# quinnchr-personal/Continuum-Mechanics-MFEM

Measured on AMD Instinct MI355X. Metric: DoF-iter/s (CG, 3D p=2 hex convection-diffusion) + achieved HBM GB/s, higher is better.
Workload: dtype f64; 1 GPU; 64x64x64 hex, H1 p=2, PA D+C+M (kinds=7), Jacobi-CG 100 it/step; dofs=2146689, elements=262144, parallelism=single, series=weak: an n^3 slab per rank

## Files before the change

continuum-mechanics-mfem_amd/csrc/brick_core.hpp:

```cpp
#pragma once
#include <hip/hip_runtime.h>

#include <cstdint>

#include "pa_core.hpp"

#ifndef CDFEM_PS8_SKIP
#define CDFEM_PS8_SKIP 1
#endif

namespace cdfem {

struct BrickGeom {
    int nbx, nby, nbz;
    int Lx, Ly, Lz;
    int xcd;
    int bz0, bzs;
    const uint8_t *bess;
    int stag = 0, stag_round = 0;
};

__device__ __forceinline__ void brick_stagger(const BrickGeom &g)
{
    if (g.stag == 0 || gridDim.x < 2u * (unsigned)g.stag_round) return;
    const unsigned wb = blockIdx.x;
    if (wb < (unsigned)g.stag_round && ((wb >> (g.stag & 15)) & 1u))
// ... 12 lines not shown
}
__device__ __forceinline__ void bstore(__amdgpu_buffer_rsrc_t r, uint32_t off, double v)
{
    __builtin_amdgcn_raw_buffer_store_b64(__builtin_bit_cast(u32x2_t, v), r, off, 0, 0);
}

template <int S, int STEP = 64>
struct PatchWalk {
    int x, y, z;
    __device__ __forceinline__ explicit PatchWalk(unsigned t) : x((int)(t % S)), y((int)((t / S) % S)), z((int)(t / (S * S))) {}
    __device__ __forceinline__ void next()
    {
        constexpr int dx = STEP % S, dy = (STEP / S) % S, dz = STEP / (S * S);
        x += dx;
        const int cx = x >= S ? 1 : 0;
        x -= S & -cx;
        y += dy + cx;
        const int cy = y >= S ? 1 : 0;
        y -= S & -cy;
        z += dz + cy;
    }
};

__device__ __forceinline__ int opaque(int v)
{
    asm volatile("" : "+v"(v));
    return v;
}

template <int S, int SZ = S>
__device__ __forceinline__ double patch_sum8(__amdgpu_buffer_rsrc_t bp, const BrickGeom &g, int gx, int gy, int gz)
{
    constexpr int s1 = S - 1, sz1 = SZ - 1;
    const int qx = min(gx / s1, g.nbx - 1), qy = min(gy / s1, g.nby - 1), qz = min(gz / sz1, g.nbz - 1);
    const int px = gx - qx * s1, py = gy - qy * s1, pz = gz - qz * sz1;
    const bool fx = px == 0 && qx > 0, fy = py == 0 && qy > 0, fz = pz == 0 && qz > 0;
    const uint32_t R = (uint32_t)g.nbx * S, A = (uint32_t)g.nby * S * R;
    const uint32_t P = (((uint32_t)qz * SZ + pz) * g.nby + qy) * S * R + (uint32_t)py * R + (uint32_t)qx * S + px;
    bool ax = true, ay = true, az = true;
    if constexpr (CDFEM_PS8_SKIP) {
        ax = __builtin_amdgcn_ballot_w64(fx) != 0;
        ay = __builtin_amdgcn_ballot_w64(fy) != 0;
        az = __builtin_amdgcn_ballot_w64(fz) != 0;
    }
    double t[8];
#pragma unroll
    for (int k = 0; k < 8; ++k) {
        const int sz = (k >> 2) & 1 ? 0 : 1, sy = (k >> 1) & 1 ? 0 : 1, sx = k & 1 ? 0 : 1;
        const bool ok = (!sx || fx) && (!sy || fy) && (!sz || fz);
        const uint32_t o = P - (uint32_t)sx - (uint32_t)sy * R - (uint32_t)sz * A;
        t[k] = 0.0;
        if ((!sx || ax) && (!sy || ay) && (!sz || az)) t[k] = bload(bp, ok ? 8u * o : kOOB);
    }
    double q = 0.0;
#pragma unroll
    for (int k = 0; k < 8; ++k) q += t[k];
    return q;
}

hipError_t launch_hobrick_um(cdfem_ctx *c, const BrickGeom &g, const double *r, const double *dinv, const double *d_old,
                             double *d_new, double *x);

struct GmPatchSrc {
    const double *pb;
    const uint8_t *ess;
    const double *x;
    BrickGeom g;
    FastDiv fdx, fdxy;
    int S;
};
bool brick_mult_pb_on(const cdfem_ctx *c);
GmPatchSrc gm_patch_src(const cdfem_ctx *c, const double *x);

}
```

continuum-mechanics-mfem_amd/csrc/brick_kernels.hip:

```cpp
#include <hip/hip_runtime.h>

#include <type_traits>
#include <vector>
#include <algorithm>
#include <cmath>

#include "cdfem_internal.hpp"
#include "brick_core.hpp"
#include "pa_core.hpp"
#include "reduce.hpp"

#ifndef CDFEM_BRICK_LDS
#define CDFEM_BRICK_LDS 1
#endif

namespace cdfem {

__device__ __forceinline__ int brick_id(const BrickGeom &g)
{
    if (!g.xcd) return blockIdx.x;
    const unsigned G = gridDim.x, b = blockIdx.x, x = b % 8, k = b / 8, q = G / 8, r = G % 8;
    return (int)(x * q + (x < r ? x : r) + k);
}

template <int S, int STEP = 64>
struct LatWalk {
    int x, y, z;
    uint32_t gid;
    __device__ __forceinline__ LatWalk(unsigned t, uint32_t g0, uint32_t Lx, uint32_t Lxy)
        : x((int)(t % S)), y((int)((t / S) % S)), z((int)(t / (S * S)))
    {
        gid = g0 + (uint32_t)x + Lx * (uint32_t)y + Lxy * (uint32_t)z;
    }
    __device__ __forceinline__ void next(uint32_t dgid, uint32_t cxd, uint32_t cyd)
    {
        constexpr int dx = STEP % S, dy = (STEP / S) % S, dz = STEP / (S * S);
        x += dx;
        const int cx = x >= S ? 1 : 0;
        x -= S & -cx;
        y += dy + cx;
        const int cy = y >= S ? 1 : 0;
        y -= S & -cy;
        z += dz + cy;
        gid += dgid + (cxd & (uint32_t)-cx) + (cyd & (uint32_t)-cy);
    }
};

__device__ __forceinline__ int bsel(bool c, int a, int b)
{
    const int m = -(int)c;
    return (a & m) | (b & ~m);
}
template <int S>
__device__ __forceinline__ int face_index(int a, int b, int c)
{
    constexpr int ring = 4 * S - 4;
    const int cap = a + S * b;
    const int mid = bsel(b == 0, a, bsel(b == S - 1, S + 2 * (S - 2) + a, S + 2 * (b - 1) + (int)(a == S - 1)));
    return bsel(c == 0, cap, bsel(c == S - 1, S * S + (S - 2) * ring + cap, S * S + (c - 1) * ring + mid));
}

template <int S>
constexpr int face_count() { return 2 * S * S + (S - 2) * (4 * S - 4); }

template <int S, int SZ = S>
__device__ __forceinline__ size_t patch_idx(const BrickGeom &g, int bx, int by, int bz, int px, int py, int pz)
{
    return ((((size_t)bz * SZ + pz) * g.nby + by) * S + py) * ((size_t)g.nbx * S) + (size_t)bx * S + px;
}

template <int B, int E, typename F>
__device__ __forceinline__ void static_for(F &&f)
{
    if constexpr (B < E) {
        f(std::integral_constant<int, B>{});
        static_for<B + 1, E>(f);
    }
}

__host__ __device__ constexpr int e2l_member(int cls, int r)
{
    const int a = cls & 1, b = (cls >> 1) & 1, c = (cls >> 2) & 1;
    const int nx = a ? 1 : 2, ny = b ? 1 : 2, nz = c ? 1 : 2;
    if (r >= nx * ny * nz) return -1;
    const int ix = r % nx, iy = (r / nx) % ny, iz = r / (nx * ny);
    const int dx = a ? 1 : 2 * ix, dy = b ? 1 : 2 * iy, dz = c ? 1 : 2 * iz;
    return dx + 3 * (dy + 3 * dz);
}

template <int D1, int S, int SY = S, int S2 = S * S>
__device__ __forceinline__ void brick_e2l(double *s_out, int o0, const double (&Y)[D1][D1][D1])
{
    if constexpr (D1 == 3) {
#pragma unroll
        for (int r = 0; r < 8; ++r) {
#pragma unroll
            for (int cls = 0; cls < 8; ++cls) {
                const int l = e2l_member(cls, r);
                if (l < 0) continue;
                const int dz = l / 9, dy = (l / 3) % 3, dx = l % 3;
// ... 325 lines not shown
                       : brick_dispatch<0>(c, x, nullptr, nullptr, y, which);
}





template <int D1, int Q1, unsigned K, int AF, int W = 1, bool XF = false, bool BF = false, bool FULL = false,
          int MX = 0>
__global__ void __launch_bounds__(64, W)
k_brick_cg(const double *__restrict__ r, const double *__restrict__ dinv,
           const double *__restrict__ d_old, double *__restrict__ d_new, double *__restrict__ q,
           double *__restrict__ face, const double *__restrict__ qd, const uint8_t *__restrict__ ess,
           const Tab<D1, Q1> T, const BrickGeom g, int zlo_shared, double *__restrict__ part,
           KrylovState *__restrict__ st, double *__restrict__ x, const double *__restrict__ upart, int nupart,
           int kk, double *__restrict__ gsum, uint32_t *__restrict__ gcnt, int grp, int nbrick)
{
    constexpr int P = D1 - 1;
    constexpr int S = kBrick * P + 1;
    constexpr int S2 = S * S, S3 = S * S * S;
    constexpr int NC = QLayout<K, 3>::nc;
    constexpr bool PAD = CDFEM_BRICK_LDS == 2 && P == 2;
    constexpr int SY = PAD ? 12 : S, SZ = PAD ? 112 : S2, PS = (S - 1) * SZ + (S - 1) * SY + S;
    constexpr bool UM = MX == 2;
    constexpr int NDE = D1 * D1 * D1;
    constexpr int UMB = UM ? (2 * PS > NDE * 64 ? 2 * PS : NDE * 64) : PS;
    __shared__ double s_in[UMB];
    __shared__ double s_out_own[UM ? 1 : PS];
    double *const s_out = UM ? s_in + PS : s_out_own;
    constexpr bool EP = AF == 2;
    constexpr bool EPL = EP && CDFEM_BRICK_LDS == 0;
    __shared__ double s_d[EPL ? S3 : 1];
    static_assert(!MX || (AF == 2 && D1 == 3), "the MFMA stages are built for the p = 2 Kronecker form");
    __shared__ double s_x[MX == 1 ? 3 * 3 * 4 * 64 : 1];
    if (st->done) return;
    brick_stagger(g);
    double beta = st->beta;
    constexpr int NPL = 16;
    double pv[NPL];
    if constexpr (BF) {
        if (kk > 0) {
            const auto bu = brsrc(upart, 8u * (uint32_t)nupart);
#pragma unroll
            for (int i = 0; i < NPL; ++i) pv[i] = bload(bu, 8u * ((uint32_t)threadIdx.x + 64u * i));
        }
    }
    const double alpha_prev = XF ? st->alpha : 0.0;
    const int t = threadIdx.x;
    const int bl = brick_id(g), nxy = g.nbx * g.nby;
    const int bz = g.bz0 + (bl / nxy) * g.bzs;
    const int b = bl % nxy + nxy * bz;
    const int bx = b % g.nbx, by = (b / g.nbx) % g.nby;
// ... 27 lines not shown
        const int gz = gz0 + pz;
        const bool in = i < S3 && (FULL || (gx0 + px < g.Lx && gy0 + py < g.Ly && gz < g.Lz));
        const uint32_t off = in ? 8u * gid : kOOB;
        rv[k] = bload(br, off);
        mv[k] = bload(bm, off);
        ov[k] = bload(bo, off);
        ev[k] = __builtin_amdgcn_raw_buffer_load_b8(be, in ? gid : kOOB, 0, 0);
        const bool writer = in && (px < S - 1 || lastx) && (py < S - 1 || lasty) && (pz < S - 1 || lastz);
        woffv[k] = writer ? off : kOOB;
        dbits |= (uint32_t)(writer && !(zlo_shared && gz == 0)) << k;
        if constexpr (XF) xv[k] = bload(bxf, woffv[k]);
    };
    auto form = [&](auto kc) {
        constexpr int k = decltype(kc)::value;
        const unsigned i = t + 64 * k;
        if (k == NI - 1 && i >= S3) return;
        const double dn = mv[k] * rv[k] + beta * ov[k];
        const bool e = ev[k] != 0;
        bstore(bd, woffv[k], dn);
        if constexpr (XF) bstore(bxf, woffv[k], xv[k] + alpha_prev * ov[k]);
        den += (e && ((dbits >> k) & 1u)) ? dn * dn : 0.0;
        const unsigned li = PAD ? liv[PAD ? k : 0] : i;
        s_in[li] = e ? 0.0 : dn;
        if constexpr (!UM) s_out[li] = 0.0;
        if constexpr (EP) {
            ebits |= (uint32_t)e << k;
            if constexpr (EPL) s_d[i] = ((dbits >> k) & 1u) ? dn : 0.0;
            else dev[EPL ? 0 : k] = ((dbits >> k) & 1u) ? dn : 0.0;
        }
    };
    static_for<0, GK>(gather);
    if constexpr (BF) {
        if (kk > 0) {
            double v = 0.0;
#pragma unroll
            for (int q = 0; q < NPL; ++q) v += pv[q];
            const double B = wave_sum(v);
            const bool stop = cg_stop_kind(st, B, kk) != kCgGoOn;
            if (b == 0 && t == 0) {
#ifdef CDFEM_DEBUG
                assert(st->iter == kk);
#endif
                cg_update_logic_at(st, B, kk);
            }
            if (stop) return;
            beta = B / st->nom;
        }
    }
    static_for<0, GK>(form);
    if constexpr (NG == 2) {
        static_for<GK, NI>(gather);
        static_for<GK, NI>(form);
    }
    __syncthreads();

    const int ex = t & 3, ey = (t >> 2) & 3, ez = t >> 4;
    const int o0 = P * ez * SZ + P * ey * SY + P * ex;
    auto xl = [&](int dz, int dy, int dx) { return s_in[o0 + dz * SZ + dy * SY + dx]; };
    double Y[D1][D1][D1];
    if constexpr (UM) {
        const int n16 = t & 15, kg = t >> 4;
        double av[2][7];
#pragma unroll
        for (int mt = 0; mt < 2; ++mt)
#pragma unroll
            for (int ks = 0; ks < 7; ++ks) av[mt][ks] = qd[(mt * 7 + ks) * 64 + t];
        const int ob0 = P * (n16 >> 2) * SY + P * (n16 & 3);
        auto node_off = [&](int j) { return (j / 9) * SZ + ((j / 3) % 3) * SY + j % 3; };
        v4d_t acc[2][4];
#pragma unroll
        for (int mt = 0; mt < 2; ++mt)
#pragma unroll
            for (int nt = 0; nt < 4; ++nt) acc[mt][nt] = v4d_t{0.0, 0.0, 0.0, 0.0};
#pragma unroll
        for (int ks = 0; ks < 7; ++ks) {
            const int j = 4 * ks + kg;
            const int jo = node_off(j < NDE ? j : 0);
#pragma unroll
            for (int nt = 0; nt < 4; ++nt) {
                const double bv = j < NDE ? s_in[P * nt * SZ + ob0 + jo] : 0.0;
#pragma unroll
                for (int mt = 0; mt < 2; ++mt)
                    acc[mt][nt] = __builtin_amdgcn_mfma_f64_16x16x4f64(av[mt][ks], bv, acc[mt][nt], 0, 0, 0);
            }
        }
#pragma unroll
        for (int mt = 0; mt < 2; ++mt)
#pragma unroll
            for (int i = 0; i < 4; ++i) {
                const int m = 16 * mt + 4 * i + kg;
                const int mo = node_off(m < NDE ? m : 0);
#pragma unroll
                for (int nt = 0; nt < 4; ++nt)
                    den += m < NDE ? s_in[P * nt * SZ + ob0 + mo] * acc[mt][nt][i] : 0.0;
            }
        __syncthreads();
        double *const yb = s_in;
#pragma unroll
        for (int mt = 0; mt < 2; ++mt)
#pragma unroll
            for (int i = 0; i < 4; ++i) {
                const int m = 16 * mt + 4 * i + kg;
                if (mt == 0 || m < NDE) {
#pragma unroll
                    for (int nt = 0; nt < 4; ++nt) yb[m * 64 + 16 * nt + n16] = acc[mt][nt][i];
                }
            }
        __syncthreads();
#pragma unroll
        for (int dz = 0; dz < D1; ++dz)
#pragma unroll
            for (int dy = 0; dy < D1; ++dy)
#pragma unroll
                for (int dx = 0; dx < D1; ++dx) Y[dz][dy][dx] = yb[((dz * D1 + dy) * D1 + dx) * 64 + t];
        __syncthreads();
#pragma unroll
        for (int k = 0; k < NI; ++k) {
            const unsigned i = t + 64 * k;
            if (k == NI - 1 && i >= S3) break;
            s_out[PAD ? liv[PAD ? k : 0] : i] = 0.0;
        }
        __syncthreads();
    } else if constexpr (MX == 1) {
        double gk[NC];
        kron_load_g<K>(q0, t, gk);
        const int row = t & 15, kq = t >> 4, qa = row >> 2, ia = row & 3;
        double av = 0.0;
        static_for<0, D1>([&](auto ic) {
            static_for<0, D1>([&](auto jc) {
                constexpr int i = decltype(ic)::value, j = decltype(jc)::value;
                const double fm = tM(T, i, j), fk = tK(T, i, j), fc = tCacc(T, i, j, 1.0, 0.0),
                             fct = tCacc(T, j, i, 1.0, 0.0);
                if (ia == i && kq == j) av = qa == 0 ? fm : qa == 1 ? fk : qa == 2 ? fc : fct;
            });
        });
#pragma unroll
        for (int dz = 0; dz < D1; ++dz)
#pragma unroll
            for (int dy = 0; dy < D1; ++dy)
#pragma unroll
                for (int dx = 0; dx < D1; ++dx) Y[dz][dy][dx] = 0.0;
#pragma unroll
        for (int jz = 0; jz < D1; ++jz) {
#pragma unroll
            for (int jy = 0; jy < D1; ++jy)
#pragma unroll
// ... 13 lines not shown
                double v[D1][5];
#pragma unroll
                for (int jy = 0; jy < D1; ++jy) {
                    const double *xr = &s_x[((jy * 3 + ix) * 4) * 64 + t];
                    kron_xcombine<K>(gk, xr[0], xr[64], xr[128], xr[192], v[jy]);
                }
                auto col = [&](int q, int jy) { return v[jy][q]; };
#pragma unroll
                for (int iy = 0; iy < D1; ++iy) {
                    double Yz[D1];
#pragma unroll
                    for (int iz = 0; iz < D1; ++iz) Yz[iz] = Y[iz][iy][ix];
                    kron_yz<D1, Q1, K>(T, gk, col, iy, jz, Yz);
#pragma unroll
                    for (int iz = 0; iz < D1; ++iz) Y[iz][iy][ix] = Yz[iz];
                }
            }
            __syncthreads();
        }
    } else {
        elem_apply3d_af<D1, Q1, K, AF>(xl, q0, t, T, Y, qd);
    }

    if constexpr (!UM) {
#pragma unroll
        for (int dz = 0; dz < D1; ++dz)
#pragma unroll
            for (int dy = 0; dy < D1; ++dy)
#pragma unroll
                for (int dx = 0; dx < D1; ++dx) den += s_in[o0 + dz * SZ + dy * SY + dx] * Y[dz][dy][dx];
    }
    brick_e2l<D1, S, SY, SZ>(s_out, o0, Y);

    {
        const uint32_t R = (uint32_t)g.nbx * S, A = (uint32_t)g.nby * S * R;
        const uint32_t base = (uint32_t)bz * S * A + (uint32_t)by * S * R + (uint32_t)bx * S;
        const auto bp = brsrc(face, 8u * (uint32_t)g.nbx * g.nby * g.nbz * S3);
        const unsigned to = (unsigned)opaque(t);
        PatchWalk<S> pw(to);
#pragma unroll
        for (int k = 0; k < NI; ++k) {
            const unsigned i = to + 64 * k;
            if (k == NI - 1 && i >= S3) break;
            double v = s_out[PAD ? (uint32_t)pw.x + SY * (uint32_t)pw.y + SZ * (uint32_t)pw.z : i];
            if constexpr (EPL) v = ((ebits >> k) & 1u) ? s_d[i] : v;
            else if constexpr (EP) v = ((ebits >> k) & 1u) ? dev[EPL ? 0 : k] : v;
            bstore(bp, 8u * (base + (uint32_t)pw.z * A + (uint32_t)pw.y * R + (uint32_t)pw.x), v);
            pw.next();
        }
    }
    den = wave_sum(den);
    if (grp <= 1) {
        if (t == 0) part[b] = den;
        return;
// ... 338 lines not shown
template <int D1, int Q1, unsigned K>
static hipError_t brick_cg2_launch(cdfem_ctx *c, const double *r, const double *dinv,
                                   const double *d_old, double *d_new, double *q, const BrickRun &run, double *x)
{
    const Tab<D1, Q1> T = make_tab<D1, Q1>(c->rule_op);
    BrickGeom g = geom_of(c);
    g.bz0 = run.bz0;
    g.bzs = run.bzs;
    const dim3 grid((unsigned)(c->nbx * c->nby * run.nlay)), block(64);
    const bool whole = run.nlay == c->nbz && run.s == c->stream;
    const double *qd = c->d_qaff ? c->d_qaff : pa_geom_on(c) ? c->d_geom : c->d_qd;
    const double *upart = c->d_part + c->nblk;
    double *const dpart = c->den_out ? c->den_out : c->d_part;
    const int grp = c->den_grp, nbrick = c->nblk;
#define CDFEM_BCG6(AFF_, W_, XF_, BF_, FU_, MX_)                                                            \
    if (whole)                                                                                               \
        CDFEM_LAUNCH(c, (k_brick_cg<D1, Q1, K, AFF_, W_, XF_, BF_, FU_, MX_>), grid, block, 0, r, dinv, d_old, d_new, q, \
                     c->d_face, qd, c->d_ess, T, g, c->zlo_shared, dpart, c->d_state, x, upart, run.nupart,     \
                     run.kk, c->d_gsum, c->d_gcnt, grp, nbrick);                                             \
    else                                                                                                     \
        hipLaunchKernelGGL((k_brick_cg<D1, Q1, K, AFF_, W_, XF_, BF_, FU_, MX_>), grid, block, 0, run.s, r, dinv, \
                           d_old, d_new, q, c->d_face, qd, c->d_ess, T, g, c->zlo_shared, dpart, c->d_state, x, \
                           upart, run.nupart, run.kk, c->d_gsum, c->d_gcnt, grp, nbrick)
    constexpr bool kMX = K == 7 && D1 == 3;
    constexpr bool kUM = (K == 7 || K == 5) && D1 == 3;
    const bool mx = kMX && c->brick_mfma != 0;
    const bool um = kUM && uniform_elem(c);
    if (um) qd = c->d_uelem;
#define CDFEM_BCG5(AFF_, W_, XF_, BF_, FU_)                                                                 \
    if constexpr (kUM && AFF_ == 2) {                                                                        \
        if (um) { CDFEM_BCG6(AFF_, W_, XF_, BF_, FU_, 2); }                                                  \
        else if (mx) { CDFEM_BCG6(AFF_, W_, XF_, BF_, FU_, (kMX ? 1 : 0)); }                                 \
        else { CDFEM_BCG6(AFF_, W_, XF_, BF_, FU_, 0); }                                                     \
    } else {                                                                                                 \
        CDFEM_BCG6(AFF_, W_, XF_, BF_, FU_, 0);                                                              \
    }
#define CDFEM_BCG4(AFF_, W_, XF_, BF_)                                                                      \
    if (full) { CDFEM_BCG5(AFF_, W_, XF_, BF_, true); } else { CDFEM_BCG5(AFF_, W_, XF_, BF_, false); }
#define CDFEM_BCG3(AFF_, W_, XF_) CDFEM_BCG5(AFF_, W_, XF_, false, false)
#define CDFEM_BCG(AFF_, W_) CDFEM_BCG3(AFF_, W_, false)
    const bool full = c->sx % kBrick == 0 && c->sy % kBrick == 0 && c->sz % kBrick == 0;
    if (pa_af(c) == 2 && run.kk >= 0) {
        if (x) { CDFEM_BCG4(2, 2, true, true); }
        else { CDFEM_BCG4(2, 2, false, true); }
    } else if (pa_af(c) == 2) {
        if (x) { CDFEM_BCG4(2, 2, true, false); }
        else { CDFEM_BCG4(2, 2, false, false); }
    } else if (pa_af(c) == 1) {
        CDFEM_BCG(1, 1);
    } else if (pa_geom_on(c)) {
        CDFEM_BCG(3, 1);
    } else {
        CDFEM_BCG(0, 1);
    }
#undef CDFEM_BCG
// ... 249 lines not shown
}

hipError_t launch_pack_qplanes(cdfem_ctx *c, const double *q, hipStream_t s)
{
    const BrickGeom g = geom_of(c);
    const int n = (int)(c->Lx * c->Ly);
    const dim3 grid((n + 255) / 256), block(256);
    if (!s) s = c->stream;
    if (c->p >= 3 && c->hb_ez != kHoBrickEdge) return hipErrorInvalidValue;
    if (c->p == 1)
        hipLaunchKernelGGL(k_pack_qplanes<kBrick * 1 + 1>, grid, block, 0, s, q, c->d_face, g,
                           c->zlo_shared, c->zhi_shared, c->d_if[0], c->d_if[2], c->d_state);
    else if (c->p == 2 || c->p == 4)
        hipLaunchKernelGGL(k_pack_qplanes<kBrick * 2 + 1>, grid, block, 0, s, q, c->d_face, g,
                           c->zlo_shared, c->zhi_shared, c->d_if[0], c->d_if[2], c->d_state);
    else if (c->p == 3)
        hipLaunchKernelGGL(k_pack_qplanes<kHoBrickEdge * 3 + 1>, grid, block, 0, s, q, c->d_face, g,
                           c->zlo_shared, c->zhi_shared, c->d_if[0], c->d_if[2], c->d_state);
    else
        return hipErrorInvalidValue;
    return hipGetLastError();
}

__global__ void __launch_bounds__(256)
k_uniform_check(const double *__restrict__ gaff, const int32_t *__restrict__ perm, int nslots, int nc, int ne,
                double tol, int *__restrict__ bad)
{
    const int s = blockIdx.x * blockDim.x + threadIdx.x;
    if (s >= nslots) return;
    const int e = perm[s];
    if (e < 0 || e >= ne) return;
    const size_t b = (size_t)(s / kLanes), lane = (size_t)(s % kLanes);
    bool diff = false;
    for (int k = 0; k < nc; ++k) diff |= fabs(gaff[(b * nc + k) * kLanes + lane] - gaff[(size_t)k * kLanes]) > tol;
    if (diff) *bad = 1;
}

template <int D1, int Q1, unsigned K>
__global__ void __launch_bounds__(64)
k_uniform_elem(const double *__restrict__ gaff, const Tab<D1, Q1> T, double *__restrict__ A)
{
    constexpr int N = D1 * D1 * D1;
    const int j = threadIdx.x;
    if (j >= N) return;
    double g[QLayout<K, 3>::nc];
    kron_load_g<K>(gaff, 0, g);
    auto xl = [&](int z, int y, int x) { return (z * D1 + y) * D1 + x == j ? 1.0 : 0.0; };
    double Y[D1][D1][D1];
    kron_core<D1, Q1, K>(xl, g, T, Y);
    for (int i = 0; i < N; ++i) A[i * N + j] = Y[i / (D1 * D1)][(i / D1) % D1][i % D1];
}

hipError_t setup_uniform_elem(cdfem_ctx *c)
{
    if (c->d_uelem) {
        const hipError_t e = hipFree(c->d_uelem);
        c->d_uelem = nullptr;
        if (e != hipSuccess) return e;
    }
    if (!c->pa_uniform || !c->structured || c->qlay != 0 || c->dim != 3 || pa_af(c) != 2 || c->p != 2 ||
        c->rule_op.q1 != 4 || c->ncomp < 1 || (c->kinds != 7 && c->kinds != 5))
        return hipSuccess;
    const int nc = c->ncomp;
    std::vector<double> g0(nc);
    hipError_t e = hipMemcpy2D(g0.data(), sizeof(double), c->d_qaff, kLanes * sizeof(double), sizeof(double), nc,
                               hipMemcpyDeviceToHost);
    if (e != hipSuccess) return e;
    double gmax = 0.0;
    for (double v : g0) gmax = std::max(gmax, std::fabs(v));
    constexpr int N = 27;
    void *scratch = nullptr;
    if ((e = hipMalloc(&scratch, sizeof(double) * (N * N + 1))) != hipSuccess) return e;
    int *bad = static_cast<int *>(scratch);
    double *A = static_cast<double *>(scratch) + 1;
    int hbad = 0;
    const int nslots = c->nblk * kLanes;
    e = hipMemsetAsync(bad, 0, sizeof(int), c->stream);
    if (e == hipSuccess) {
        hipLaunchKernelGGL(k_uniform_check, dim3((nslots + 255) / 256), dim3(256), 0, c->stream, c->d_qaff, c->d_perm,
                           nslots, nc, (int)c->ne, 1e-14 * gmax, bad);
        e = hipGetLastError();
    }
    if (e == hipSuccess) e = hipMemcpyAsync(&hbad, bad, sizeof(int), hipMemcpyDeviceToHost, c->stream);
    if (e == hipSuccess) e = hipStreamSynchronize(c->stream);
    std::vector<double> h(N * N), op(2 * 7 * 64, 0.0);
    if (e == hipSuccess && !hbad) {
        const Tab<3, 4> T = make_tab<3, 4>(c->rule_op);
        if (c->kinds == 7) hipLaunchKernelGGL((k_uniform_elem<3, 4, 7>), dim3(1), dim3(64), 0, c->stream, c->d_qaff, T, A);
        else hipLaunchKernelGGL((k_uniform_elem<3, 4, 5>), dim3(1), dim3(64), 0, c->stream, c->d_qaff, T, A);
        e = hipGetLastError();
        if (e == hipSuccess) e = hipMemcpyAsync(h.data(), A, sizeof(double) * N * N, hipMemcpyDeviceToHost, c->stream);
        if (e == hipSuccess) e = hipStreamSynchronize(c->stream);
    }
    const hipError_t ef = hipFree(scratch);
    if (e != hipSuccess) return e;
    if (ef != hipSuccess) return ef;
    if (hbad) return hipSuccess;
    for (int mt = 0; mt < 2; ++mt)
        for (int ks = 0; ks < 7; ++ks)
            for (int l = 0; l < 64; ++l) {
                const int i = 16 * mt + (l & 15), j = 4 * ks + (l >> 4);
                op[(mt * 7 + ks) * 64 + l] = (i < N && j < N) ? h[i * N + j] : 0.0;
            }
    void *d = nullptr;
    if ((e = hipMalloc(&d, sizeof(double) * op.size())) != hipSuccess) return e;
    e = hipMemcpy(d, op.data(), sizeof(double) * op.size(), hipMemcpyHostToDevice);
    if (e != hipSuccess) {
        (void)hipFree(d);
        return e;
    }
    c->d_uelem = static_cast<double *>(d);
    return hipSuccess;
}

}
```

Baseline: 40.28 billion DoF-iter/s.

## Split uniform-element MFMA brick CG into dedicated kernel with class-ordered row permutation

Moves the uniform-element path (one dense 27x27 element matrix applied with f64 MFMA) out of the generic brick CG kernel into its own kernel file. The element matrix rows are permuted so that each group of four MFMA output rows covers distinct parity classes, letting results scatter into shared memory without write conflicts and without the extra staging pass through shared memory that the old path used. The new kernel has fixed launch bounds of two waves per SIMD and its own LDS layout. It adds code duplication, and the new scatter scheme has to accumulate contributions correctly without atomics.

```diff
diff --git a/continuum-mechanics-mfem_amd/csrc/brick_core.hpp b/continuum-mechanics-mfem_amd/csrc/brick_core.hpp
--- a/continuum-mechanics-mfem_amd/csrc/brick_core.hpp
+++ b/continuum-mechanics-mfem_amd/csrc/brick_core.hpp
@@ -2,6 +2,7 @@
 #include <hip/hip_runtime.h>
 
 #include <cstdint>
+#include <type_traits>
 
 #include "pa_core.hpp"
 
@@ -60,6 +61,45 @@
     }
 };
 
+__device__ __forceinline__ int brick_id(const BrickGeom &g)
+{
+    if (!g.xcd) return blockIdx.x;
+    const unsigned G = gridDim.x, b = blockIdx.x, x = b % 8, k = b / 8, q = G / 8, r = G % 8;
+    return (int)(x * q + (x < r ? x : r) + k);
+}
+
+template <int S, int STEP = 64>
+struct LatWalk {
+    int x, y, z;
+    uint32_t gid;
+    __device__ __forceinline__ LatWalk(unsigned t, uint32_t g0, uint32_t Lx, uint32_t Lxy)
+        : x((int)(t % S)), y((int)((t / S) % S)), z((int)(t / (S * S)))
+    {
+        gid = g0 + (uint32_t)x + Lx * (uint32_t)y + Lxy * (uint32_t)z;
+    }
+    __device__ __forceinline__ void next(uint32_t dgid, uint32_t cxd, uint32_t cyd)
+    {
+        constexpr int dx = STEP % S, dy = (STEP / S) % S, dz = STEP / (S * S);
+        x += dx;
+        const int cx = x >= S ? 1 : 0;
+        x -= S & -cx;
+        y += dy + cx;
+        const int cy = y >= S ? 1 : 0;
+        y -= S & -cy;
+        z += dz + cy;
+        gid += dgid + (cxd & (uint32_t)-cx) + (cyd & (uint32_t)-cy);
+    }
+};
+
+template <int B, int E, typename F>
+__device__ __forceinline__ void static_for(F &&f)
+{
+    if constexpr (B < E) {
+        f(std::integral_constant<int, B>{});
+        static_for<B + 1, E>(f);
+    }
+}
+
 __device__ __forceinline__ int opaque(int v)
 {
     asm volatile("" : "+v"(v));
@@ -99,6 +139,10 @@
 hipError_t launch_hobrick_um(cdfem_ctx *c, const BrickGeom &g, const double *r, const double *dinv, const double *d_old,
                              double *d_new, double *x);
 
+hipError_t launch_brick_um(cdfem_ctx *c, const BrickGeom &g, unsigned nbrick_launch, hipStream_t s, bool whole,
+                           const double *r, const double *dinv, const double *d_old, double *d_new, double *x, int kk,
+                           int nupart);
+
 struct GmPatchSrc {
     const double *pb;
     const uint8_t *ess;
diff --git a/continuum-mechanics-mfem_amd/csrc/brick_kernels.hip b/continuum-mechanics-mfem_amd/csrc/brick_kernels.hip
--- a/continuum-mechanics-mfem_amd/csrc/brick_kernels.hip
+++ b/continuum-mechanics-mfem_amd/csrc/brick_kernels.hip
@@ -16,36 +16,6 @@
 
 namespace cdfem {
 
-__device__ __forceinline__ int brick_id(const BrickGeom &g)
-{
-    if (!g.xcd) return blockIdx.x;
-    const unsigned G = gridDim.x, b = blockIdx.x, x = b % 8, k = b / 8, q = G / 8, r = G % 8;
-    return (int)(x * q + (x < r ? x : r) + k);
-}
-
-template <int S, int STEP = 64>
-struct LatWalk {
-    int x, y, z;
-    uint32_t gid;
-    __device__ __forceinline__ LatWalk(unsigned t, uint32_t g0, uint32_t Lx, uint32_t Lxy)
-        : x((int)(t % S)), y((int)((t / S) % S)), z((int)(t / (S * S)))
-    {
-        gid = g0 + (uint32_t)x + Lx * (uint32_t)y + Lxy * (uint32_t)z;
-    }
-    __device__ __forceinline__ void next(uint32_t dgid, uint32_t cxd, uint32_t cyd)
-    {
-        constexpr int dx = STEP % S, dy = (STEP / S) % S, dz = STEP / (S * S);
-        x += dx;
-        const int cx = x >= S ? 1 : 0;
-        x -= S & -cx;
-        y += dy + cx;
-        const int cy = y >= S ? 1 : 0;
-        y -= S & -cy;
-        z += dz + cy;
-        gid += dgid + (cxd & (uint32_t)-cx) + (cyd & (uint32_t)-cy);
-    }
-};
-
 __device__ __forceinline__ int bsel(bool c, int a, int b)
 {
     const int m = -(int)c;
@@ -67,15 +37,6 @@
 __device__ __forceinline__ size_t patch_idx(const BrickGeom &g, int bx, int by, int bz, int px, int py, int pz)
 {
     return ((((size_t)bz * SZ + pz) * g.nby + by) * S + py) * ((size_t)g.nbx * S) + (size_t)bx * S + px;
-}
-
-template <int B, int E, typename F>
-__device__ __forceinline__ void static_for(F &&f)
-{
-    if constexpr (B < E) {
-        f(std::integral_constant<int, B>{});
-        static_for<B + 1, E>(f);
-    }
 }
 
 __host__ __device__ constexpr int e2l_member(int cls, int r)
@@ -447,12 +408,8 @@
     constexpr int NC = QLayout<K, 3>::nc;
     constexpr bool PAD = CDFEM_BRICK_LDS == 2 && P == 2;
     constexpr int SY = PAD ? 12 : S, SZ = PAD ? 112 : S2, PS = (S - 1) * SZ + (S - 1) * SY + S;
-    constexpr bool UM = MX == 2;
-    constexpr int NDE = D1 * D1 * D1;
-    constexpr int UMB = UM ? (2 * PS > NDE * 64 ? 2 * PS : NDE * 64) : PS;
-    __shared__ double s_in[UMB];
-    __shared__ double s_out_own[UM ? 1 : PS];
-    double *const s_out = UM ? s_in + PS : s_out_own;
+    __shared__ double s_in[PS];
+    __shared__ double s_out[PS];
     constexpr bool EP = AF == 2;
     constexpr bool EPL = EP && CDFEM_BRICK_LDS == 0;
     __shared__ double s_d[EPL ? S3 : 1];
@@ -526,7 +483,7 @@
         den += (e && ((dbits >> k) & 1u)) ? dn * dn : 0.0;
         const unsigned li = PAD ? liv[PAD ? k : 0] : i;
         s_in[li] = e ? 0.0 : dn;
-        if constexpr (!UM) s_out[li] = 0.0;
+        s_out[li] = 0.0;
         if constexpr (EP) {
             ebits |= (uint32_t)e << k;
             if constexpr (EPL) s_d[i] = ((dbits >> k) & 1u) ? dn : 0.0;
@@ -562,70 +519,7 @@
     const int o0 = P * ez * SZ + P * ey * SY + P * ex;
     auto xl = [&](int dz, int dy, int dx) { return s_in[o0 + dz * SZ + dy * SY + dx]; };
     double Y[D1][D1][D1];
-    if constexpr (UM) {
-        const int n16 = t & 15, kg = t >> 4;
-        double av[2][7];
-#pragma unroll
-        for (int mt = 0; mt < 2; ++mt)
-#pragma unroll
-            for (int ks = 0; ks < 7; ++ks) av[mt][ks] = qd[(mt * 7 + ks) * 64 + t];
-        const int ob0 = P * (n16 >> 2) * SY + P * (n16 & 3);
-        auto node_off = [&](int j) { return (j / 9) * SZ + ((j / 3) % 3) * SY + j % 3; };
-        v4d_t acc[2][4];
-#pragma unroll
-        for (int mt = 0; mt < 2; ++mt)
-#pragma unroll
-            for (int nt = 0; nt < 4; ++nt) acc[mt][nt] = v4d_t{0.0, 0.0, 0.0, 0.0};
-#pragma unroll
-        for (int ks = 0; ks < 7; ++ks) {
-            const int j = 4 * ks + kg;
-            const int jo = node_off(j < NDE ? j : 0);
-#pragma unroll
-            for (int nt = 0; nt < 4; ++nt) {
-                const double bv = j < NDE ? s_in[P * nt * SZ + ob0 + jo] : 0.0;
-#pragma unroll
-                for (int mt = 0; mt < 2; ++mt)
-                    acc[mt][nt] = __builtin_amdgcn_mfma_f64_16x16x4f64(av[mt][ks], bv, acc[mt][nt], 0, 0, 0);
-            }
-        }
-#pragma unroll
-        for (int mt = 0; mt < 2; ++mt)
-#pragma unroll
-            for (int i = 0; i < 4; ++i) {
-                const int m = 16 * mt + 4 * i + kg;
-                const int mo = node_off(m < NDE ? m : 0);
-#pragma unroll
-                for (int nt = 0; nt < 4; ++nt)
-                    den += m < NDE ? s_in[P * nt * SZ + ob0 + mo] * acc[mt][nt][i] : 0.0;
-            }
-        __syncthreads();
-        double *const yb = s_in;
-#pragma unroll
-        for (int mt = 0; mt < 2; ++mt)
-#pragma unroll
-            for (int i = 0; i < 4; ++i) {
-                const int m = 16 * mt + 4 * i + kg;
-                if (mt == 0 || m < NDE) {
-#pragma unroll
-                    for (int nt = 0; nt < 4; ++nt) yb[m * 64 + 16 * nt + n16] = acc[mt][nt][i];
-                }
-            }
-        __syncthreads();
-#pragma unroll
-        for (int dz = 0; dz < D1; ++dz)
-#pragma unroll
-            for (int dy = 0; dy < D1; ++dy)
-#pragma unroll
-                for (int dx = 0; dx < D1; ++dx) Y[dz][dy][dx] = yb[((dz * D1 + dy) * D1 + dx) * 64 + t];
-        __syncthreads();
-#pragma unroll
-        for (int k = 0; k < NI; ++k) {
-            const unsigned i = t + 64 * k;
-            if (k == NI - 1 && i >= S3) break;
-            s_out[PAD ? liv[PAD ? k : 0] : i] = 0.0;
-        }
-        __syncthreads();
-    } else if constexpr (MX == 1) {
+    if constexpr (MX == 1) {
         double gk[NC];
         kron_load_g<K>(q0, t, gk);
         const int row = t & 15, kq = t >> 4, qa = row >> 2, ia = row & 3;
@@ -685,14 +579,12 @@
         elem_apply3d_af<D1, Q1, K, AF>(xl, q0, t, T, Y, qd);
     }
 
-    if constexpr (!UM) {
-#pragma unroll
-        for (int dz = 0; dz < D1; ++dz)
-#pragma unroll
-            for (int dy = 0; dy < D1; ++dy)
-#pragma unroll
-                for (int dx = 0; dx < D1; ++dx) den += s_in[o0 + dz * SZ + dy * SY + dx] * Y[dz][dy][dx];
-    }
+#pragma unroll
+    for (int dz = 0; dz < D1; ++dz)
+#pragma unroll
+        for (int dy = 0; dy < D1; ++dy)
+#pragma unroll
+            for (int dx = 0; dx < D1; ++dx) den += s_in[o0 + dz * SZ + dy * SY + dx] * Y[dz][dy][dx];
     brick_e2l<D1, S, SY, SZ>(s_out, o0, Y);
 
     {
@@ -1077,15 +969,15 @@
         hipLaunchKernelGGL((k_brick_cg<D1, Q1, K, AFF_, W_, XF_, BF_, FU_, MX_>), grid, block, 0, run.s, r, dinv, \
                            d_old, d_new, q, c->d_face, qd, c->d_ess, T, g, c->zlo_shared, dpart, c->d_state, x, \
                            upart, run.nupart, run.kk, c->d_gsum, c->d_gcnt, grp, nbrick)
+    if constexpr ((K == 7 || K == 5) && D1 == 3) {
+        if (uniform_elem(c))
+            return launch_brick_um(c, g, grid.x, run.s, whole, r, dinv, d_old, d_new, x, run.kk, run.nupart);
+    }
     constexpr bool kMX = K == 7 && D1 == 3;
-    constexpr bool kUM = (K == 7 || K == 5) && D1 == 3;
     const bool mx = kMX && c->brick_mfma != 0;
-    const bool um = kUM && uniform_elem(c);
-    if (um) qd = c->d_uelem;
 #define CDFEM_BCG5(AFF_, W_, XF_, BF_, FU_)                                                                 \
-    if constexpr (kUM && AFF_ == 2) {                                                                        \
-        if (um) { CDFEM_BCG6(AFF_, W_, XF_, BF_, FU_, 2); }                                                  \
-        else if (mx) { CDFEM_BCG6(AFF_, W_, XF_, BF_, FU_, (kMX ? 1 : 0)); }                                 \
+    if constexpr (kMX && AFF_ == 2) {                                                                        \
+        if (mx) { CDFEM_BCG6(AFF_, W_, XF_, BF_, FU_, 1); }                                                  \
         else { CDFEM_BCG6(AFF_, W_, XF_, BF_, FU_, 0); }                                                     \
     } else {                                                                                                 \
         CDFEM_BCG6(AFF_, W_, XF_, BF_, FU_, 0);                                                              \
@@ -1381,95 +1273,4 @@
     return hipGetLastError();
 }
 
-__global__ void __launch_bounds__(256)
-k_uniform_check(const double *__restrict__ gaff, const int32_t *__restrict__ perm, int nslots, int nc, int ne,
-                double tol, int *__restrict__ bad)
-{
-    const int s = blockIdx.x * blockDim.x + threadIdx.x;
-    if (s >= nslots) return;
-    const int e = perm[s];
-    if (e < 0 || e >= ne) return;
-    const size_t b = (size_t)(s / kLanes), lane = (size_t)(s % kLanes);
-    bool diff = false;
-    for (int k = 0; k < nc; ++k) diff |= fabs(gaff[(b * nc + k) * kLanes + lane] - gaff[(size_t)k * kLanes]) > tol;
-    if (diff) *bad = 1;
-}
-
-template <int D1, int Q1, unsigned K>
-__global__ void __launch_bounds__(64)
-k_uniform_elem(const double *__restrict__ gaff, const Tab<D1, Q1> T, double *__restrict__ A)
-{
-    constexpr int N = D1 * D1 * D1;
-    const int j = threadIdx.x;
-    if (j >= N) return;
-    double g[QLayout<K, 3>::nc];
-    kron_load_g<K>(gaff, 0, g);
-    auto xl = [&](int z, int y, int x) { return (z * D1 + y) * D1 + x == j ? 1.0 : 0.0; };
-    double Y[D1][D1][D1];
-    kron_core<D1, Q1, K>(xl, g, T, Y);
-    for (int i = 0; i < N; ++i) A[i * N + j] = Y[i / (D1 * D1)][(i / D1) % D1][i % D1];
-}
-
-hipError_t setup_uniform_elem(cdfem_ctx *c)
-{
-    if (c->d_uelem) {
-        const hipError_t e = hipFree(c->d_uelem);
-        c->d_uelem = nullptr;
-        if (e != hipSuccess) return e;
-    }
-    if (!c->pa_uniform || !c->structured || c->qlay != 0 || c->dim != 3 || pa_af(c) != 2 || c->p != 2 ||
-        c->rule_op.q1 != 4 || c->ncomp < 1 || (c->kinds != 7 && c->kinds != 5))
-        return hipSuccess;
-    const int nc = c->ncomp;
-    std::vector<double> g0(nc);
-    hipError_t e = hipMemcpy2D(g0.data(), sizeof(double), c->d_qaff, kLanes * sizeof(double), sizeof(double), nc,
-                               hipMemcpyDeviceToHost);
-    if (e != hipSuccess) return e;
-    double gmax = 0.0;
-    for (double v : g0) gmax = std::max(gmax, std::fabs(v));
-    constexpr int N = 27;
-    void *scratch = nullptr;
-    if ((e = hipMalloc(&scratch, sizeof(double) * (N * N + 1))) != hipSuccess) return e;
-    int *bad = static_cast<int *>(scratch);
-    double *A = static_cast<double *>(scratch) + 1;
-    int hbad = 0;
-    const int nslots = c->nblk * kLanes;
-    e = hipMemsetAsync(bad, 0, sizeof(int), c->stream);
-    if (e == hipSuccess) {
-        hipLaunchKernelGGL(k_uniform_check, dim3((nslots + 255) / 256), dim3(256), 0, c->stream, c->d_qaff, c->d_perm,
-                           nslots, nc, (int)c->ne, 1e-14 * gmax, bad);
-        e = hipGetLastError();
-    }
-    if (e == hipSuccess) e = hipMemcpyAsync(&hbad, bad, sizeof(int), hipMemcpyDeviceToHost, c->stream);
-    if (e == hipSuccess) e = hipStreamSynchronize(c->stream);
-    std::vector<double> h(N * N), op(2 * 7 * 64, 0.0);
-    if (e == hipSuccess && !hbad) {
-        const Tab<3, 4> T = make_tab<3, 4>(c->rule_op);
-        if (c->kinds == 7) hipLaunchKernelGGL((k_uniform_elem<3, 4, 7>), dim3(1), dim3(64), 0, c->stream, c->d_qaff, T, A);
-        else hipLaunchKernelGGL((k_uniform_elem<3, 4, 5>), dim3(1), dim3(64), 0, c->stream, c->d_qaff, T, A);
-        e = hipGetLastError();
-        if (e == hipSuccess) e = hipMemcpyAsync(h.data(), A, sizeof(double) * N * N, hipMemcpyDeviceToHost, c->stream);
-        if (e == hipSuccess) e = hipStreamSynchronize(c->stream);
-    }
-    const hipError_t ef = hipFree(scratch);
-    if (e != hipSuccess) return e;
-    if (ef != hipSuccess) return ef;
-    if (hbad) return hipSuccess;
-    for (int mt = 0; mt < 2; ++mt)
-        for (int ks = 0; ks < 7; ++ks)
-            for (int l = 0; l < 64; ++l) {
-                const int i = 16 * mt + (l & 15), j = 4 * ks + (l >> 4);
-                op[(mt * 7 + ks) * 64 + l] = (i < N && j < N) ? h[i * N + j] : 0.0;
-            }
-    void *d = nullptr;
-    if ((e = hipMalloc(&d, sizeof(double) * op.size())) != hipSuccess) return e;
-    e = hipMemcpy(d, op.data(), sizeof(double) * op.size(), hipMemcpyHostToDevice);
-    if (e != hipSuccess) {
-        (void)hipFree(d);
-        return e;
-    }
-    c->d_uelem = static_cast<double *>(d);
-    return hipSuccess;
-}
-
-}
+}
diff --git a/continuum-mechanics-mfem_amd/csrc/brick_um.hip b/continuum-mechanics-mfem_amd/csrc/brick_um.hip
--- /dev/null
+++ b/continuum-mechanics-mfem_amd/csrc/brick_um.hip
@@ -0,0 +1,380 @@
+#include <hip/hip_runtime.h>
+
+#include <algorithm>
+#include <cmath>
+#include <vector>
+
+#include "cdfem_internal.hpp"
+#include "brick_core.hpp"
+#include "pa_core.hpp"
+#include "reduce.hpp"
+
+#ifndef CDFEM_BUM_ADD
+#define CDFEM_BUM_ADD 0
+#endif
+
+namespace cdfem {
+
+constexpr int kUmSlots = 32, kUmN = 27;
+constexpr int kUmRow[kUmSlots] = {0,  1,  4,  3,  2,  7,  22, 5,  6,  19, 10, 21, 8,  25, 16, 23,
+                                  18, 9,  12, 13, 20, 11, 14, -1, 24, 15, -1, -1, 26, 17, -1, -1};
+constexpr int um_class(int l) { return (l % 3 & 1) | ((l / 3 % 3 & 1) << 1) | ((l / 9 & 1) << 2); }
+constexpr bool um_row_order_ok()
+{
+    int seen[kUmN] = {};
+    for (int g = 0; g < kUmSlots / 4; ++g) {
+        int cls = 0;
+        if (kUmRow[4 * g] < 0 || um_class(kUmRow[4 * g]) != 0) return false;
+        for (int k = 0; k < 4; ++k) {
+            const int l = kUmRow[4 * g + k];
+            if (l < 0) continue;
+            if (l >= kUmN || seen[l]++) return false;
+            if (cls & (1 << um_class(l))) return false;
+            cls |= 1 << um_class(l);
+        }
+    }
+    for (int l = 0; l < kUmN; ++l)
+        if (!seen[l]) return false;
+    return true;
+}
+static_assert(um_row_order_ok(), "kUmRow: every dof once, one class once per group of 4 slots");
+
+template <int G>
+__device__ __forceinline__ int um_slot_off(int kg)
+{
+    constexpr int S = 9;
+    auto off = [](int l) constexpr { return l < 0 ? -1 : (l / 9) * S * S + (l / 3 % 3) * S + l % 3; };
+    constexpr int o0 = off(kUmRow[4 * G]), o1 = off(kUmRow[4 * G + 1]), o2 = off(kUmRow[4 * G + 2]),
+                  o3 = off(kUmRow[4 * G + 3]);
+    return kg == 0 ? o0 : kg == 1 ? o1 : kg == 2 ? o2 : o3;
+}
+template <int G>
+constexpr bool um_group_padded() { return kUmRow[4 * G + 1] < 0 || kUmRow[4 * G + 2] < 0 || kUmRow[4 * G + 3] < 0; }
+
+template <bool XF, bool BF, bool FULL>
+__global__ void __launch_bounds__(64, 2)
+k_brick_cg(const double *__restrict__ r, const double *__restrict__ dinv, const double *__restrict__ d_old,
+           double *__restrict__ d_new, double *__restrict__ face, const double *__restrict__ amat,
+           const uint8_t *__restrict__ ess, const BrickGeom g, int zlo_shared, double *__restrict__ part,
+           KrylovState *__restrict__ st, double *__restrict__ x, const double *__restrict__ upart, int nupart,
+           int kk, double *__restrict__ gsum, uint32_t *__restrict__ gcnt, int grp, int nbrick)
+{
+    constexpr int P = 2, S = kBrick * P + 1, S2 = S * S, S3 = S * S * S, NDE = kUmN;
+    static_assert(S == 9, "um_slot_off is written for the 9^3 patch");
+    __shared__ double s_in[S3];
+    __shared__ double s_out[S3];
+    if (st->done) return;
+    brick_stagger(g);
+    double beta = st->beta;
+    constexpr int NPL = 16;
+    double pv[NPL];
+    if constexpr (BF) {
+        if (kk > 0) {
+            const auto bu = brsrc(upart, 8u * (uint32_t)nupart);
+#pragma unroll
+            for (int i = 0; i < NPL; ++i) pv[i] = bload(bu, 8u * ((uint32_t)threadIdx.x + 64u * i));
+        }
+    }
+    const double alpha_prev = XF ? st->alpha : 0.0;
+    const int t = threadIdx.x;
+    const int bl = brick_id(g), nxy = g.nbx * g.nby;
+    const int bz = g.bz0 + (bl / nxy) * g.bzs;
+    const int b = bl % nxy + nxy * bz;
+    const int bx = b % g.nbx, by = (b / g.nbx) % g.nby;
+    const int gx0 = (S - 1) * bx, gy0 = (S - 1) * by, gz0 = (S - 1) * bz;
+    const bool lastx = bx == g.nbx - 1, lasty = by == g.nby - 1, lastz = bz == g.nbz - 1;
+    double den = 0.0;
+    constexpr int NI = (S3 + 63) / 64;
+    const int Lx = g.Lx, Lxy = g.Lx * g.Ly;
+    const uint32_t nl = (uint32_t)Lxy * (uint32_t)g.Lz;
+    const auto br = brsrc(r, 8u * nl), bm = brsrc(dinv, 8u * nl), bo = brsrc(d_old, 8u * nl);
+    const auto be = brsrc(ess, nl), bd = brsrc(d_new, 8u * nl), bxf = brsrc(x, XF ? 8u * nl : 0u);
+    double rv[NI], mv[NI], ov[NI], xv[NI];
+    uint32_t woffv[NI];
+    uint32_t dbits = 0, ebits = 0;
+    uint8_t ev[NI];
+    double dev[NI];
+    const uint32_t uLx = (uint32_t)Lx, uLxy = (uint32_t)Lxy;
+    constexpr uint32_t wdx = 64 % S, wdy = (64 / S) % S, wdz = 64 / (S * S);
+    const uint32_t dgid = wdx + wdy * uLx + wdz * uLxy, cxd = uLx - S, cyd = uLxy - S * uLx;
+    LatWalk<S> pw0(t, (uint32_t)gx0 + uLx * (uint32_t)gy0 + uLxy * (uint32_t)gz0, uLx, uLxy);
+    auto gather = [&](auto kc) {
+        constexpr int k = decltype(kc)::value;
+        const unsigned i = t + 64 * k;
+        const int px = pw0.x, py = pw0.y, pz = pw0.z;
+        const uint32_t gid = pw0.gid;
+        pw0.next(dgid, cxd, cyd);
+        const int gz = gz0 + pz;
+        const bool in = i < S3 && (FULL || (gx0 + px < g.Lx && gy0 + py < g.Ly && gz < g.Lz));
+        const uint32_t off = in ? 8u * gid : kOOB;
+        rv[k] = bload(br, off);
+        mv[k] = bload(bm, off);
+        ov[k] = bload(bo, off);
+        ev[k] = __builtin_amdgcn_raw_buffer_load_b8(be, in ? gid : kOOB, 0, 0);
+        const bool writer = in && (px < S - 1 || lastx) && (py < S - 1 || lasty) && (pz < S - 1 || lastz);
+        woffv[k] = writer ? off : kOOB;
+        dbits |= (uint32_t)(writer && !(zlo_shared && gz == 0)) << k;
+        if constexpr (XF) xv[k] = bload(bxf, woffv[k]);
+    };
+    auto form = [&](auto kc) {
+        constexpr int k = decltype(kc)::value;
+        const unsigned i = t + 64 * k;
+        if (k == NI - 1 && i >= S3) return;
+        const double dn = mv[k] * rv[k] + beta * ov[k];
+        const bool e = ev[k] != 0;
+        bstore(bd, woffv[k], dn);
+        if constexpr (XF) bstore(bxf, woffv[k], xv[k] + alpha_prev * ov[k]);
+        den += (e && ((dbits >> k) & 1u)) ? dn * dn : 0.0;
+        s_in[i] = e ? 0.0 : dn;
+        s_out[i] = 0.0;
+        ebits |= (uint32_t)e << k;
+        dev[k] = ((dbits >> k) & 1u) ? dn : 0.0;
+    };
+    static_for<0, NI>(gather);
+    if constexpr (BF) {
+        if (kk > 0) {
+            double v = 0.0;
+#pragma unroll
+            for (int q = 0; q < NPL; ++q) v += pv[q];
+            const double B = wave_sum(v);
+            const bool stop = cg_stop_kind(st, B, kk) != kCgGoOn;
+            if (b == 0 && t == 0) {
+#ifdef CDFEM_DEBUG
+                assert(st->iter == kk);
+#endif
+                cg_update_logic_at(st, B, kk);
+            }
+            if (stop) return;
+            beta = B / st->nom;
+        }
+    }
+    static_for<0, NI>(form);
+    __syncthreads();
+
+    {
+        const int n16 = t & 15, kg = t >> 4;
+        double av[2][7];
+#pragma unroll
+        for (int mt = 0; mt < 2; ++mt)
+#pragma unroll
+            for (int ks = 0; ks < 7; ++ks) av[mt][ks] = amat[(mt * 7 + ks) * 64 + t];
+        const int ob0 = P * (n16 >> 2) * S + P * (n16 & 3);
+        const bool vxy = FULL || (gx0 + P * (n16 & 3) + P < g.Lx && gy0 + P * (n16 >> 2) + P < g.Ly);
+        auto node_off = [&](int j) { return (j / 9) * S2 + ((j / 3) % 3) * S + j % 3; };
+        v4d_t acc[2][4];
+#pragma unroll
+        for (int mt = 0; mt < 2; ++mt)
+#pragma unroll
+            for (int nt = 0; nt < 4; ++nt) acc[mt][nt] = v4d_t{0.0, 0.0, 0.0, 0.0};
+#pragma unroll
+        for (int ks = 0; ks < 7; ++ks) {
+            const int j = 4 * ks + kg;
+            const int jo = node_off(j < NDE ? j : 0);
+#pragma unroll
+            for (int nt = 0; nt < 4; ++nt) {
+                const bool ok = j < NDE && vxy && (FULL || gz0 + P * nt + P < g.Lz);
+                const double xin = s_in[P * nt * S2 + ob0 + jo];
+                const double bv = ok ? xin : 0.0;
+#pragma unroll
+                for (int mt = 0; mt < 2; ++mt)
+                    acc[mt][nt] = __builtin_amdgcn_mfma_f64_16x16x4f64(av[mt][ks], bv, acc[mt][nt], 0, 0, 0);
+            }
+        }
+        static_for<0, 8>([&](auto gc) {
+            constexpr int G = decltype(gc)::value, mt = G / 4, i = G % 4;
+            constexpr bool PADG = um_group_padded<G>();
+            const int so = um_slot_off<G>(kg);
+            const bool live = !PADG || so >= 0;
+            const int o = ob0 + (PADG ? max(so, 0) : so);
+#pragma unroll
+            for (int nt = 0; nt < 4; ++nt) {
+                const double xin = s_in[P * nt * S2 + o];
+                den += live ? xin * acc[mt][nt][i] : 0.0;
+            }
+            if (live) {
+#if CDFEM_BUM_ADD == 1
+#pragma unroll
+                for (int nt = 0; nt < 4; ++nt)
+                    (void)__hip_atomic_fetch_add(&s_out[P * nt * S2 + o], acc[mt][nt][i], __ATOMIC_RELAXED,
+                                                 __HIP_MEMORY_SCOPE_WORKGROUP);
+#else
+#pragma unroll
+                for (int h = 0; h < 2; ++h) {
+                    double *const p0 = &s_out[P * h * S2 + o], *const p1 = &s_out[P * (h + 2) * S2 + o];
+                    const double v0 = *p0, v1 = *p1;
+                    *p0 = v0 + acc[mt][h][i];
+                    *p1 = v1 + acc[mt][h + 2][i];
+                }
+#endif
+            }
+        });
+    }
+    __syncthreads();
+
+    {
+        const uint32_t R = (uint32_t)g.nbx * S, A = (uint32_t)g.nby * S * R;
+        const uint32_t base = (uint32_t)bz * S * A + (uint32_t)by * S * R + (uint32_t)bx * S;
+        const auto bp = brsrc(face, 8u * (uint32_t)g.nbx * g.nby * g.nbz * S3);
+        const unsigned to = (unsigned)opaque(t);
+        PatchWalk<S> pw(to);
+#pragma unroll
+        for (int k = 0; k < NI; ++k) {
+            const unsigned i = to + 64 * k;
+            if (k == NI - 1 && i >= S3) break;
+            double v = s_out[i];
+            v = ((ebits >> k) & 1u) ? dev[k] : v;
+            bstore(bp, 8u * (base + (uint32_t)pw.z * A + (uint32_t)pw.y * R + (uint32_t)pw.x), v);
+            pw.next();
+        }
+    }
+    den = wave_sum(den);
+    if (grp <= 1) {
+        if (t == 0) part[b] = den;
+        return;
+    }
+    const int gi = b / grp, g0 = gi * grp, gn = min(grp, nbrick - g0);
+    uint32_t prev = 0;
+    if (t == 0) {
+        __hip_atomic_store(&part[b], den, __ATOMIC_RELAXED, __HIP_MEMORY_SCOPE_AGENT);
+        asm volatile("s_waitcnt vmcnt(0)" ::: "memory");
+        prev = __hip_atomic_fetch_add(&gcnt[gi], 1u, __ATOMIC_RELAXED, __HIP_MEMORY_SCOPE_AGENT);
+    }
+    prev = (uint32_t)__shfl((int)prev, 0, 64);
+    if (prev != (uint32_t)(gn - 1)) return;
+    double v = t < gn ? __hip_atomic_load(&part[g0 + t], __ATOMIC_RELAXED, __HIP_MEMORY_SCOPE_AGENT) : 0.0;
+    v = wave_sum(v);
+    if (t == 0) {
+        gsum[gi] = v;
+        __hip_atomic_store(&gcnt[gi], 0u, __ATOMIC_RELAXED, __HIP_MEMORY_SCOPE_AGENT);
+    }
+}
+
+hipError_t launch_brick_um(cdfem_ctx *c, const BrickGeom &g, unsigned nbrick_launch, hipStream_t s, bool whole,
+                           const double *r, const double *dinv, const double *d_old, double *d_new, double *x, int kk,
+                           int nupart)
+{
+    if (c->d_uelem == nullptr || c->p != 2) return hipErrorInvalidValue;
+    const dim3 grid(nbrick_launch), block(64);
+    const double *upart = c->d_part + c->nblk;
+    double *const dpart = c->den_out ? c->den_out : c->d_part;
+    const bool full = c->sx % kBrick == 0 && c->sy % kBrick == 0 && c->sz % kBrick == 0;
+#define CDFEM_BUM(XF_, BF_, FU_)                                                                              \
+    do {                                                                                                      \
+        if (whole)                                                                                            \
+            CDFEM_LAUNCH(c, (k_brick_cg<XF_, BF_, FU_>), grid, block, 0, r, dinv, d_old, d_new, c->d_face,      \
+                         c->d_uelem, c->d_ess, g, c->zlo_shared, dpart, c->d_state, x, upart, nupart, kk,       \
+                         c->d_gsum, c->d_gcnt, c->den_grp, c->nblk);                                            \
+        else                                                                                                  \
+            hipLaunchKernelGGL((k_brick_cg<XF_, BF_, FU_>), grid, block, 0, s, r, dinv, d_old, d_new, c->d_face, \
+                               c->d_uelem, c->d_ess, g, c->zlo_shared, dpart, c->d_state, x, upart, nupart, kk, \
+                               c->d_gsum, c->d_gcnt, c->den_grp, c->nblk);                                      \
+    } while (0)
+#define CDFEM_BUM2(XF_, BF_)                                                                                  \
+    do {                                                                                                      \
+        if (full) CDFEM_BUM(XF_, BF_, true);                                                                  \
+        else CDFEM_BUM(XF_, BF_, false);                                                                      \
+    } while (0)
+    if (kk >= 0) {
+        if (x) CDFEM_BUM2(true, true);
+        else CDFEM_BUM2(false, true);
+    } else {
+        if (x) CDFEM_BUM2(true, false);
+        else CDFEM_BUM2(false, false);
+    }
+#undef CDFEM_BUM2
+#undef CDFEM_BUM
+    return hipGetLastError();
+}
+
+__global__ void __launch_bounds__(256)
+k_uniform_check(const double *__restrict__ gaff, const int32_t *__restrict__ perm, int nslots, int nc, int ne,
+                double tol, int *__restrict__ bad)
+{
+    const int s = blockIdx.x * blockDim.x + threadIdx.x;
+    if (s >= nslots) return;
+    const int e = perm[s];
+    if (e < 0 || e >= ne) return;
+    const size_t b = (size_t)(s / kLanes), lane = (size_t)(s % kLanes);
+    bool diff = false;
+    for (int k = 0; k < nc; ++k) diff |= fabs(gaff[(b * nc + k) * kLanes + lane] - gaff[(size_t)k * kLanes]) > tol;
+    if (diff) *bad = 1;
+}
+
+template <int D1, int Q1, unsigned K>
+__global__ void __launch_bounds__(64)
+k_uniform_elem(const double *__restrict__ gaff, const Tab<D1, Q1> T, double *__restrict__ A)
+{
+    constexpr int N = D1 * D1 * D1;
+    const int j = threadIdx.x;
+    if (j >= N) return;
+    double g[QLayout<K, 3>::nc];
+    kron_load_g<K>(gaff, 0, g);
+    auto xl = [&](int z, int y, int x) { return (z * D1 + y) * D1 + x == j ? 1.0 : 0.0; };
+    double Y[D1][D1][D1];
+    kron_core<D1, Q1, K>(xl, g, T, Y);
+    for (int i = 0; i < N; ++i) A[i * N + j] = Y[i / (D1 * D1)][(i / D1) % D1][i % D1];
+}
+
+hipError_t setup_uniform_elem(cdfem_ctx *c)
+{
+    if (c->d_uelem) {
+        const hipError_t e = hipFree(c->d_uelem);
+        c->d_uelem = nullptr;
+        if (e != hipSuccess) return e;
+    }
+    if (!c->pa_uniform || !c->structured || c->qlay != 0 || c->dim != 3 || pa_af(c) != 2 || c->p != 2 ||
+        c->rule_op.q1 != 4 || c->ncomp < 1 || (c->kinds != 7 && c->kinds != 5))
+        return hipSuccess;
+    const int nc = c->ncomp;
+    std::vector<double> g0(nc);
+    hipError_t e = hipMemcpy2D(g0.data(), sizeof(double), c->d_qaff, kLanes * sizeof(double), sizeof(double), nc,
+                               hipMemcpyDeviceToHost);
+    if (e != hipSuccess) return e;
+    double gmax = 0.0;
+    for (double v : g0) gmax = std::max(gmax, std::fabs(v));
+    constexpr int N = kUmN;
+    void *scratch = nullptr;
+    if ((e = hipMalloc(&scratch, sizeof(double) * (N * N + 1))) != hipSuccess) return e;
+    int *bad = static_cast<int *>(scratch);
+    double *A = static_cast<double *>(scratch) + 1;
+    int hbad = 0;
+    const int nslots = c->nblk * kLanes;
+    e = hipMemsetAsync(bad, 0, sizeof(int), c->stream);
+    if (e == hipSuccess) {
+        hipLaunchKernelGGL(k_uniform_check, dim3((nslots + 255) / 256), dim3(256), 0, c->stream, c->d_qaff, c->d_perm,
+                           nslots, nc, (int)c->ne, 1e-14 * gmax, bad);
+        e = hipGetLastError();
+    }
+    if (e == hipSuccess) e = hipMemcpyAsync(&hbad, bad, sizeof(int), hipMemcpyDeviceToHost, c->stream);
+    if (e == hipSuccess) e = hipStreamSynchronize(c->stream);
+    std::vector<double> h(N * N), op(2 * 7 * 64, 0.0);
+    if (e == hipSuccess && !hbad) {
+        const Tab<3, 4> T = make_tab<3, 4>(c->rule_op);
+        if (c->kinds == 7) hipLaunchKernelGGL((k_uniform_elem<3, 4, 7>), dim3(1), dim3(64), 0, c->stream, c->d_qaff, T, A);
+        else hipLaunchKernelGGL((k_uniform_elem<3, 4, 5>), dim3(1), dim3(64), 0, c->stream, c->d_qaff, T, A);
+        e = hipGetLastError();
+        if (e == hipSuccess) e = hipMemcpyAsync(h.data(), A, sizeof(double) * N * N, hipMemcpyDeviceToHost, c->stream);
+        if (e == hipSuccess) e = hipStreamSynchronize(c->stream);
+    }
+    const hipError_t ef = hipFree(scratch);
+    if (e != hipSuccess) return e;
+    if (ef != hipSuccess) return ef;
+    if (hbad) return hipSuccess;
+    for (int mt = 0; mt < 2; ++mt)
+        for (int ks = 0; ks < 7; ++ks)
+            for (int l = 0; l < 64; ++l) {
+                const int i = kUmRow[16 * mt + (l & 15)], j = 4 * ks + (l >> 4);
+                op[(mt * 7 + ks) * 64 + l] = (i >= 0 && j < N) ? h[i * N + j] : 0.0;
+            }
+    void *d = nullptr;
+    if ((e = hipMalloc(&d, sizeof(double) * op.size())) != hipSuccess) return e;
+    e = hipMemcpy(d, op.data(), sizeof(double) * op.size(), hipMemcpyHostToDevice);
+    if (e != hipSuccess) {
+        (void)hipFree(d);
+        return e;
+    }
+    c->d_uelem = static_cast<double *>(d);
+    return hipSuccess;
+}
+
+}
```

Measured after the change: 43.24 billion DoF-iter/s (median of 6 runs). 1.07x the previous value.
